# ilyakurdyukov/jpeg-quantsmooth

Hardware: AMD Instinct MI355X
Metric: 8x8 blocks/s at q=3 niter=3 (higher is better)
Workload: dtype f32

## Files before the change

### jpeg-quantsmooth_amd/csrc/qs_kernels.hip

```cpp
#include <hip/hip_runtime.h>
#include <stdint.h>
#include <stdlib.h>
#include "qs_device.h"
#include "qs_devfn.h"



__device__ __forceinline__ void wave_lds_sync() {
  __builtin_amdgcn_fence(__ATOMIC_RELEASE, "wavefront");
  __builtin_amdgcn_wave_barrier();
  __builtin_amdgcn_fence(__ATOMIC_ACQUIRE, "wavefront");
}

__device__ __forceinline__ uint32_t mulc(uint32_t a, int c) {
  return (uint32_t)__mul24((int)a, c);
}

__device__ __forceinline__ uint32_t lshl13_add(uint32_t x, uint32_t b) {
  uint32_t r;
  asm("v_lshl_add_u32 %0, %1, 13, %2" : "=v"(r) : "v"(x), "v"(b));
  return r;
}

__device__ __forceinline__ void idct8(uint32_t (&v)[8], uint32_t bias) {
  uint32_t z1, z2, z3, z4, z5, t0, t1, t2, t3, e0, e1, e2, e3;
  z2 = v[2]; z3 = v[6];
  z1 = mulc(z2 + z3, 4433);
  asm volatile("" : "+v"(z1));
  t2 = z1 - mulc(z3, 15137);
  t3 = z1 + mulc(z2, 6270);
  t0 = lshl13_add(v[0] + v[4], bias);
  t1 = lshl13_add(v[0] - v[4], bias);
  e0 = t0 + t3; e3 = t0 - t3; e1 = t1 + t2; e2 = t1 - t2;
  t0 = v[7]; t1 = v[5]; t2 = v[3]; t3 = v[1];
  z1 = t0 + t3; z2 = t1 + t2; z3 = t0 + t2; z4 = t1 + t3;
  z5 = mulc(z3 + z4, 9633);
  asm volatile("" : "+v"(z5));
  t0 = mulc(t0, 2446);  t1 = mulc(t1, 16819);
  t2 = mulc(t2, 25172); t3 = mulc(t3, 12299);
  z1 = mulc(z1, 7373);  z2 = mulc(z2, 20995);
  z3 = mulc(z3, 16069); z4 = mulc(z4, 3196);
  z3 = z5 - z3; z4 = z5 - z4;
  t0 += z3 - z1; t1 += z4 - z2; t2 += z3 - z2; t3 += z4 - z1;
  v[0] = e0 + t3; v[7] = e0 - t3;
  v[1] = e1 + t2; v[6] = e1 - t2;
  v[2] = e2 + t1; v[5] = e2 - t1;
  v[3] = e3 + t0; v[4] = e3 - t0;
}

__device__ __forceinline__ void idct_pass1(uint32_t (&ws)[64]) {
#pragma unroll
  for (int x = 0; x < 8; ++x) {
    uint32_t col[8];
#pragma unroll
    for (int j = 0; j < 8; ++j) col[j] = ws[j * 8 + x];
    idct8(col, 1024u);
#pragma unroll
    for (int j = 0; j < 8; ++j) ws[j * 8 + x] = (uint32_t)((int32_t)col[j] >> 11);
  }
}

__device__ __forceinline__ void idct_pass2_row(uint32_t (&row)[8], int (&out)[8]) {
  idct8(row, 257u << 17);
#pragma unroll
  for (int j = 0; j < 8; ++j) {
    int z = (int32_t)row[j];
    z = min(max(z, 0), (256 << 18) - 1);
    out[j] = z >> 18;
  }
}

#define QS_PIX_BITS 0x45000000u
__device__ __forceinline__ void idct_pass2_row_f(uint32_t (&row)[8], float (&out)[8]) {
  idct8(row, 257u << 17);
#pragma unroll
  for (int j = 0; j < 8; ++j) {
    int z = (int32_t)row[j];
    z = min(max(z, 0), (256 << 18) - 1);
    out[j] = __builtin_bit_cast(float, __builtin_amdgcn_alignbit(QS_PIX_BITS >> 14, (uint32_t)z, 18));
  }
}
__device__ __forceinline__ float pix_from_byte(uint32_t v, int n) {
  return __builtin_bit_cast(float, QS_PIX_BITS | ((v >> (8 * n)) & 0xffu));
}

__device__ __forceinline__ void
store_pixel_row(uint8_t* __restrict__ org, int pitch, int y, const int (&o)[8], int bx, int by, int wblk, int hblk,
                int rep_top, int rep_bot) {
  uint2 pk;
  pk.x = (uint32_t)o[0] | ((uint32_t)o[1] << 8) | ((uint32_t)o[2] << 16) | ((uint32_t)o[3] << 24);
  pk.y = (uint32_t)o[4] | ((uint32_t)o[5] << 8) | ((uint32_t)o[6] << 16) | ((uint32_t)o[7] << 24);
  uint8_t* rp = org + (size_t)y * pitch;
  *reinterpret_cast<uint2*>(rp) = pk;
  const bool top = (y == 0 && by == 0 && rep_top), bot = (y == 7 && by == hblk - 1 && rep_bot);
  if (bx == 0) {
    rp[-1] = (uint8_t)o[0];
    if (top) rp[-1 - pitch] = (uint8_t)o[0];
    if (bot) rp[-1 + pitch] = (uint8_t)o[0];
  }
  if (bx == wblk - 1) {
    rp[8] = (uint8_t)o[7];
    if (top) rp[8 - pitch] = (uint8_t)o[7];
    if (bot) rp[8 + pitch] = (uint8_t)o[7];
  }
  if (top) *reinterpret_cast<uint2*>(rp - pitch) = pk;
  if (bot) *reinterpret_cast<uint2*>(rp + pitch) = pk;
}

__device__ __forceinline__ void
idct_ws_to_plane(uint32_t (&ws)[64], uint8_t* __restrict__ plane, int wblk, int hblk, int pitch,
                 int rep_top, int rep_bot, int blk) {
  const int by = blk / wblk, bx = blk - by * wblk;
  idct_pass1(ws);
  uint8_t* org = plane + (size_t)(by * 8 + 1) * pitch + QS_APRON_X + bx * 8;
#pragma unroll
  for (int y = 0; y < 8; ++y) {
    uint32_t row[8]; int o[8];
#pragma unroll
    for (int j = 0; j < 8; ++j) row[j] = ws[y * 8 + j];
    idct_pass2_row(row, o);
    store_pixel_row(org, pitch, y, o, bx, by, wblk, hblk, rep_top, rep_bot);
  }
}

__device__ __forceinline__ void
idct_wave_to_plane(const QsConsts* __restrict__ cst, int16_t* __restrict__ coef,
                   uint8_t* __restrict__ plane, int wblk, int hblk, int pitch,
                   int first, int defer, int rep_top, int rep_bot, int* __restrict__ status, int base, uint32_t* lds) {
  const int lane = threadIdx.x & 63;
  const int nblk = wblk * hblk;
  const int nvec = min(64, nblk - base) * 8;
  uint4* gsrc = reinterpret_cast<uint4*>(coef) + (size_t)base * 8;
  uint4 v[8];
#pragma unroll
  for (int j = 0; j < 8; ++j) {
    const int idx = j * 64 + lane;
    v[j] = make_uint4(0, 0, 0, 0);
    if (idx < nvec) v[j] = gsrc[idx];
  }
  if (first) {
    int q[8], bad = 0;
    qs_load_qraw8(cst, lane & 7, q);
#pragma unroll
    for (int j = 0; j < 8; ++j) v[j] = qs_dequant8<true>(v[j], q, bad);
    if (!defer) {
#pragma unroll
      for (int j = 0; j < 8; ++j) {
        const int idx = j * 64 + lane;
        if (idx < nvec) gsrc[idx] = v[j];
      }
    }
    if (bad) atomicOr(status, 1);
  }
  {
    const int m0 = (lane & 7) * 4;
#pragma unroll
    for (int j = 0; j < 8; ++j) {
      uint32_t* dst = lds + m0 * QS_LDS_PITCH + (j * 8 + (lane >> 3));
      dst[0] = v[j].x; dst[QS_LDS_PITCH] = v[j].y; dst[2 * QS_LDS_PITCH] = v[j].z; dst[3 * QS_LDS_PITCH] = v[j].w;
    }
  }
  wave_lds_sync();
  const uint32_t* col = lds + lane;
  uint32_t ws[64];
#pragma unroll
  for (int r = 0; r < 32; ++r) {
    const uint32_t d = col[r * QS_LDS_PITCH];
    ws[r * 2] = (uint32_t)(int32_t)(int16_t)(d & 0xffff);
    ws[r * 2 + 1] = (uint32_t)((int32_t)d >> 16);
  }
  if (base + lane < nblk) idct_ws_to_plane(ws, plane, wblk, hblk, pitch, rep_top, rep_bot, base + lane);
}

__global__ void __launch_bounds__(256)
qs_idct_plane_kernel(const QsConsts* __restrict__ cst, int16_t* __restrict__ coef,
                     uint8_t* __restrict__ plane, int wblk, int hblk, int pitch,
                     int first, int rep_top, int rep_bot, int* __restrict__ status) {
  __shared__ uint32_t lds_all[4][32 * QS_LDS_PITCH];
  const int wave = threadIdx.x >> 6;
  const int base = __builtin_amdgcn_readfirstlane((int)(blockIdx.x * 256 + wave * 64));
  if (base >= wblk * hblk) return;
  idct_wave_to_plane(cst, coef, plane, wblk, hblk, pitch, first & 1, first & 2, rep_top, rep_bot, status, base, lds_all[wave]);
}

__global__ void __launch_bounds__(256)
qs_idct_set_kernel(const QsPlaneSet set, int first) {
  __shared__ uint32_t lds_all[4][32 * QS_LDS_PITCH];
  const int wave = threadIdx.x >> 6;
  const int w = __builtin_amdgcn_readfirstlane((int)(blockIdx.x * 4 + wave));
  if (w >= set.wave0[set.n]) return;
  const int i = qs_set_find(set, w);
  const QsPlaneRef& r = set.ref[i];
  const int base = (w - set.wave0[i]) * 64;
  if (base >= r.wblk * r.hblk) return;
  idct_wave_to_plane(r.cst, r.coef, r.plane, r.wblk, r.hblk, r.pitch, first, r.mode & QS_PLANE_QUANT,
                     r.mode & QS_PLANE_REP_TOP, r.mode & QS_PLANE_REP_BOT, r.status, base, lds_all[wave]);
}



typedef int16_t __attribute__((may_alias)) lds_i16;
__device__ __forceinline__ int lds_coef(const uint32_t* col, int i) {
  const lds_i16* p = reinterpret_cast<const lds_i16*>(col + (i >> 1) * QS_LDS_PITCH) + (i & 1);
  return *p;
}
__device__ __forceinline__ void lds_set_coef(uint32_t* col, int i, int v) {
  lds_i16* p = reinterpret_cast<lds_i16*>(col + (i >> 1) * QS_LDS_PITCH) + (i & 1);
  *p = (lds_i16)v;
}

static_assert(QS_LDS_PITCH * 4 == 260, "the literal offsets below assume a 260-byte row pitch");
#define QS_LDS16_GROUP(BASE, W, N0, O) \
  asm volatile("ds_read_i16 %0, %16 offset:" #O "\n\tds_read_i16 %1, %16 offset:" #O "+2\n\t" \
               "ds_read_i16 %2, %16 offset:" #O "+260\n\tds_read_i16 %3, %16 offset:" #O "+262\n\t" \
               "ds_read_i16 %4, %16 offset:" #O "+520\n\tds_read_i16 %5, %16 offset:" #O "+522\n\t" \
               "ds_read_i16 %6, %16 offset:" #O "+780\n\tds_read_i16 %7, %16 offset:" #O "+782\n\t" \
               "ds_read_i16 %8, %16 offset:" #O "+1040\n\tds_read_i16 %9, %16 offset:" #O "+1042\n\t" \
               "ds_read_i16 %10, %16 offset:" #O "+1300\n\tds_read_i16 %11, %16 offset:" #O "+1302\n\t" \
               "ds_read_i16 %12, %16 offset:" #O "+1560\n\tds_read_i16 %13, %16 offset:" #O "+1562\n\t" \
               "ds_read_i16 %14, %16 offset:" #O "+1820\n\tds_read_i16 %15, %16 offset:" #O "+1822\n\t" \
               "s_waitcnt lgkmcnt(0)" \
               : "=&v"(W[(N0) + 0]), "=&v"(W[(N0) + 1]), "=&v"(W[(N0) + 2]), "=&v"(W[(N0) + 3]), \
                 "=&v"(W[(N0) + 4]), "=&v"(W[(N0) + 5]), "=&v"(W[(N0) + 6]), "=&v"(W[(N0) + 7]), \
                 "=&v"(W[(N0) + 8]), "=&v"(W[(N0) + 9]), "=&v"(W[(N0) + 10]), "=&v"(W[(N0) + 11]), \
                 "=&v"(W[(N0) + 12]), "=&v"(W[(N0) + 13]), "=&v"(W[(N0) + 14]), "=&v"(W[(N0) + 15]) \
               : "v"(BASE) : "memory")
__device__ __forceinline__ void lds_read_block_i16(const uint32_t* col, uint32_t (&ws)[64]) {
  typedef const __attribute__((address_space(3))) uint32_t* lds_ptr;
  const uint32_t a0 = (uint32_t)(uintptr_t)(lds_ptr)col;
  const uint32_t a1 = a0 + 8 * 260, a2 = a0 + 16 * 260, a3 = a0 + 24 * 260;
  QS_LDS16_GROUP(a0, ws, 0, 0);
  QS_LDS16_GROUP(a1, ws, 16, 0);
  QS_LDS16_GROUP(a2, ws, 32, 0);
  QS_LDS16_GROUP(a3, ws, 48, 0);
}
__device__ __forceinline__ void lds_read_block_i16_1(const uint32_t* col, uint32_t (&ws)[64]) {
  typedef const __attribute__((address_space(3))) uint32_t* lds_ptr;
  const uint32_t a0 = (uint32_t)(uintptr_t)(lds_ptr)col;
  QS_LDS16_GROUP(a0, ws, 0, 0);
  QS_LDS16_GROUP(a0, ws, 16, 2080);
  QS_LDS16_GROUP(a0, ws, 32, 4160);
  QS_LDS16_GROUP(a0, ws, 48, 6240);
}

#define QS_PIX_SCALE 0.000244140625f
#define QS_TERM_D(D, W) { \
    float u_ = __builtin_amdgcn_fmed3f(Rs - __builtin_fabsf(D), 0.0f, 1.0f); \
    float t_ = u_ * u_; \
    float x_ = (D) * t_; \
    float y_ = (W) * t_; \
    num = num + x_ * y_; \
    den = den + y_ * y_; }
#define QS_TERM(A, B, W) { float d_ = (A) - (B); QS_TERM_D(d_, W) }

typedef float qs_w16 __attribute__((ext_vector_type(16)));
typedef int qs_i4 __attribute__((ext_vector_type(4)));
#define QS_SWAIT(BUF) asm volatile("s_waitcnt lgkmcnt(0)" : "+s"(BUF) : : "memory")

#define QS_WAVES_PER_WG 4
#define QS_SMOOTH_MIN_WAVES 3
#define QS_RESIDENT_WG (256 * QS_SMOOTH_MIN_WAVES * 4 / QS_WAVES_PER_WG)
#define QS_PRIO_SLOW 3
#define QS_PRIO_TERMS 0

#define QS_TERM_OPT(COND, A, B, W) { float d_, t_; \
        asm volatile( \
          "s_cmp_lg_u32 %[c], 0\n\t" \
          "s_cbranch_scc1 1f\n\t" \
          "v_sub_f32 %[d], %[a], %[b]\n\t" \
          "v_sub_f32 %[t], %[r], |%[d]| clamp\n\t" \
          "v_mul_f32 %[t], %[t], %[t]\n\t" \
          "v_mul_f32 %[d], %[d], %[t]\n\t" \
          "v_mul_f32 %[t], %[w], %[t]\n\t" \
          "v_mul_f32 %[d], %[d], %[t]\n\t" \
          "v_add_f32 %[n], %[n], %[d]\n\t" \
          "v_mul_f32 %[d], %[t], %[t]\n\t" \
          "v_add_f32 %[e], %[e], %[d]\n" \
          "1:" \
          : [n] "+v"(num), [e] "+v"(den), [d] "=&v"(d_), [t] "=&v"(t_) \
          : [a] "v"(A), [b] "v"(B), [w] "s"(W), [r] "s"(Rs), [c] "s"(COND) : "scc"); }
#define QS_TERM_ASM(A, B, W) { float d_, t_; \
        asm volatile( \
          "v_sub_f32 %[d], %[a], %[b]\n\t" \
          "v_sub_f32 %[t], %[r], |%[d]| clamp\n\t" \
          "v_mul_f32 %[t], %[t], %[t]\n\t" \
          "v_mul_f32 %[d], %[d], %[t]\n\t" \
          "v_mul_f32 %[t], %[w], %[t]\n\t" \
          "v_mul_f32 %[d], %[d], %[t]\n\t" \
          "v_add_f32 %[n], %[n], %[d]\n\t" \
          "v_mul_f32 %[d], %[t], %[t]\n\t" \
          "v_add_f32 %[e], %[e], %[d]" \
          : [n] "+v"(num), [e] "+v"(den), [d] "=&v"(d_), [t] "=&v"(t_) \
          : [a] "v"(A), [b] "v"(B), [w] "s"(W), [r] "s"(Rs)); }

#define QS_TERM_D_ASM(D, W) { float d_, t_; \
        asm volatile( \
          "v_sub_f32 %[t], %[r], |%[a]| clamp\n\t" \
          "v_mul_f32 %[t], %[t], %[t]\n\t" \
          "v_mul_f32 %[d], %[a], %[t]\n\t" \
          "v_mul_f32 %[t], %[w], %[t]\n\t" \
          "v_mul_f32 %[d], %[d], %[t]\n\t" \
          "v_add_f32 %[n], %[n], %[d]\n\t" \
          "v_mul_f32 %[d], %[t], %[t]\n\t" \
          "v_add_f32 %[e], %[e], %[d]" \
          : [n] "+v"(num), [e] "+v"(den), [d] "=&v"(d_), [t] "=&v"(t_) \
          : [a] "v"(D), [w] "s"(W), [r] "s"(Rs)); }
#ifndef QS_HOIST_DIAG
#define QS_HOIST_DIAG 32
#endif
#ifndef QS_Q1_SKIP
#define QS_Q1_SKIP 1
#endif
#ifndef QS_STASH
#define QS_STASH 1
#endif
#define QS_X_STASH 0
#define QS_X_EDGE 8
#define QS_X_REB 16
#define QS_X_DWORDS 20
static_assert(QS_WAVES_PER_WG * (32 * QS_LDS_PITCH + QS_X_DWORDS * 64) * 4 <= 160 * 1024 / 3, "LDS budget of three workgroups per CU");
typedef unsigned long long __attribute__((address_space(3))) qs_lds_u64;
__device__ __forceinline__ void qs_lds_add64(qs_lds_u64* p, long long v) {
  __hip_atomic_fetch_add(p, (unsigned long long)v, __ATOMIC_RELAXED, __HIP_MEMORY_SCOPE_WAVEFRONT);
}
__device__ __forceinline__ qs_lds_u64* qs_xreb(const uint32_t* col, const uint32_t* lds, int n) {
  typedef const __attribute__((address_space(3))) uint32_t* lds_ptr;
  uint32_t a = (uint32_t)(uintptr_t)(lds_ptr)col;
  asm volatile("" : "+v"(a));
  const uint32_t b = (uint32_t)(uintptr_t)(lds_ptr)lds;
  return (qs_lds_u64*)(a * 2u - b + (uint32_t)((32 * QS_LDS_PITCH + (QS_X_REB + 2 * n) * 64) * 4));
}

#define QS_SMOOTH_KERNEL_NAME qs_smooth_plane_kernel
#include "qs_smooth_kernel.inc"
#undef QS_SMOOTH_KERNEL_NAME
#define QS_SMOOTH_KERNEL_NAME qs_smooth_set_kernel
#define QS_SMOOTH_SET 1
#include "qs_smooth_kernel.inc"
#undef QS_SMOOTH_KERNEL_NAME
#undef QS_SMOOTH_SET

#define QS_DP_KERNEL_NAME qs_smooth_dp_kernel
#include "qs_smooth_dp_kernel.inc"
#undef QS_DP_KERNEL_NAME
#define QS_DP_KERNEL_NAME qs_smooth_dp_set_kernel
#define QS_DP_SET 1
#include "qs_smooth_dp_kernel.inc"
#undef QS_DP_KERNEL_NAME
#undef QS_DP_SET

__global__ void __launch_bounds__(256)
qs_clamp_kernel(int16_t* __restrict__ coef, size_t nvec) {
  size_t i = (size_t)blockIdx.x * 256 + threadIdx.x;
  const size_t stride = (size_t)gridDim.x * 256;
  uint4* p = reinterpret_cast<uint4*>(coef);
  for (; i < nvec; i += stride) {
    uint4 v = p[i];
    uint32_t d[4] = {v.x, v.y, v.z, v.w};
#pragma unroll
    for (int c = 0; c < 4; ++c) {
      int lo = (int16_t)(d[c] & 0xffff), hi = (int32_t)d[c] >> 16;
      lo = min(max(lo, -1023), 1023); hi = min(max(hi, -1023), 1023);
      d[c] = ((uint32_t)lo & 0xffffu) | ((uint32_t)hi << 16);
    }
    p[i] = make_uint4(d[0], d[1], d[2], d[3]);
  }
}

__global__ void __launch_bounds__(256)
qs_dequant_kernel(const QsConsts* __restrict__ cst, int16_t* __restrict__ coef, size_t nvec) {
  size_t i = (size_t)blockIdx.x * 256 + threadIdx.x;
  const size_t stride = (size_t)gridDim.x * 256;
  uint4* p = reinterpret_cast<uint4*>(coef);
  for (; i < nvec; i += stride) {
    uint4 v = p[i];
    uint32_t d[4] = {v.x, v.y, v.z, v.w};
    const int j = (int)(i & 7);
#pragma unroll
    for (int c = 0; c < 4; ++c) {
      int lo = (int16_t)(d[c] & 0xffff), hi = (int32_t)d[c] >> 16;
      lo *= cst->qraw[j * 8 + c * 2]; hi *= cst->qraw[j * 8 + c * 2 + 1];
      d[c] = ((uint32_t)lo & 0xffffu) | ((uint32_t)hi << 16);
    }
    p[i] = make_uint4(d[0], d[1], d[2], d[3]);
  }
}

#include "qs_launch.h"

void qs_launch_idct_plane(const QsConsts* cst, int16_t* coef, uint8_t* plane, int wblk, int hblk,
                          int first, int rep_top, int rep_bot, int* status, hipStream_t s) {
  const int nblk = wblk * hblk;
  const int f = first == 3 ? 3 : first ? 1 : 0;
  hipLaunchKernelGGL(qs_idct_plane_kernel, dim3((nblk + 255) / 256), dim3(256), 0, s,
                     cst, coef, plane, wblk, hblk, qs_plane_pitch(wblk), f, rep_top, rep_bot, status);
}

#define QS_DP_WAVES 4
static int qs_dp_waves(int groups) {
  static const int on = [] { const char* v = getenv("QS_HIP_DP"); return v ? atoi(v) : 1; }();
  static const int lim = [] { const char* v = getenv("QS_HIP_DP_GROUPS"); return v ? atoi(v) : 768; }();
  static const int lim2 = [] { const char* v = getenv("QS_HIP_DP_GROUPS2"); return v ? atoi(v) : 1536; }();
  if (!on) return 0;
  return groups <= lim ? QS_DP_WAVES : groups <= lim2 ? 2 : 0;
}

void qs_launch_smooth_plane(const QsConsts* cst, int16_t* coef, const uint8_t* plane, uint8_t* plane_next, int rep_top, int rep_bot,
                            int wblk, int hblk, int diag, int rebalance, int final_clamp, int blk_begin, int blk_end, hipStream_t s) {
  const int n = blk_end - blk_begin;
  if (n <= 0) return;
  const int pitch = qs_plane_pitch(wblk);
  const int rep = (rep_top ? QS_PLANE_REP_TOP : 0) | (rep_bot ? QS_PLANE_REP_BOT : 0);
  if (const int nw = qs_dp_waves((n + 63) / 64)) {
    const dim3 g((n + 63) / 64), b(64 * nw);
#define QS_GO_DP(D, W) hipLaunchKernelGGL((qs_smooth_dp_kernel<D, W>), g, b, 0, s, cst, coef, plane, plane_next, rep, wblk, hblk, pitch, rebalance, final_clamp, blk_begin, blk_end)
    if (nw == 2) { if (diag) QS_GO_DP(true, 2); else QS_GO_DP(false, 2); }
    else if (diag) QS_GO_DP(true, QS_DP_WAVES); else QS_GO_DP(false, QS_DP_WAVES);
#undef QS_GO_DP
    return;
  }
  const int per_wg = 64 * QS_WAVES_PER_WG;
  const dim3 grid((n + per_wg - 1) / per_wg), block(per_wg);
#define QS_GO(K) hipLaunchKernelGGL(K, grid, block, 0, s, cst, coef, plane, plane_next, rep, wblk, hblk, pitch, rebalance, final_clamp, blk_begin, blk_end)
  if (diag) QS_GO(qs_smooth_plane_kernel<true>); else QS_GO(qs_smooth_plane_kernel<false>);
#undef QS_GO
}

void qs_launch_idct_set(const QsPlaneSet& set, int first, hipStream_t s) {
  const int nw = set.wave0[set.n];
  if (nw <= 0) return;
  hipLaunchKernelGGL(qs_idct_set_kernel, dim3((nw + 3) / 4), dim3(256), 0, s, set, first);
}

void qs_launch_smooth_set(const QsPlaneSet& set, int diag, int final_clamp, hipStream_t s) {
  const int nw = set.wave0[set.n];
  if (nw <= 0) return;
  if (const int dw = qs_dp_waves(nw)) {
    const dim3 g(nw), b(64 * dw);
#define QS_GO_DP(D, W) hipLaunchKernelGGL((qs_smooth_dp_set_kernel<D, W>), g, b, 0, s, set, final_clamp)
    if (dw == 2) { if (diag) QS_GO_DP(true, 2); else QS_GO_DP(false, 2); }
    else if (diag) QS_GO_DP(true, QS_DP_WAVES); else QS_GO_DP(false, QS_DP_WAVES);
#undef QS_GO_DP
    return;
  }
  const dim3 grid((nw + QS_WAVES_PER_WG - 1) / QS_WAVES_PER_WG), block(64 * QS_WAVES_PER_WG);
  if (diag) hipLaunchKernelGGL(qs_smooth_set_kernel<true>, grid, block, 0, s, set, final_clamp);
  else      hipLaunchKernelGGL(qs_smooth_set_kernel<false>, grid, block, 0, s, set, final_clamp);
}

void qs_launch_clamp(int16_t* coef, size_t nblk, hipStream_t s) {
  const size_t nvec = nblk * 8;
  const int grid = (int)((nvec + 255) / 256 < 8192 ? (nvec + 255) / 256 : 8192);
  hipLaunchKernelGGL(qs_clamp_kernel, dim3(grid ? grid : 1), dim3(256), 0, s, coef, nvec);
}

void qs_launch_dequant(const QsConsts* cst, int16_t* coef, size_t nblk, hipStream_t s) {
  const size_t nvec = nblk * 8;
  const int grid = (int)((nvec + 255) / 256 < 8192 ? (nvec + 255) / 256 : 8192);
  hipLaunchKernelGGL(qs_dequant_kernel, dim3(grid ? grid : 1), dim3(256), 0, s, cst, coef, nvec);
}
```

### jpeg-quantsmooth_amd/csrc/qs_smooth_kernel.inc

```
template <bool DIAG>
__global__ void __launch_bounds__(64 * QS_WAVES_PER_WG, QS_SMOOTH_MIN_WAVES)
#ifdef QS_SMOOTH_SET
QS_SMOOTH_KERNEL_NAME(const QsPlaneSet set, int final_clamp) {
  __shared__ __attribute__((aligned(16))) uint32_t lds_all[QS_WAVES_PER_WG][32 * QS_LDS_PITCH + (DIAG ? 0 : QS_X_DWORDS * 64)];
#if QS_STASH
  __shared__ uint32_t stash_all[QS_WAVES_PER_WG][2 * 8 * 64];
#endif
  const int lane = threadIdx.x & 63, wave = DIAG ? (int)(threadIdx.x >> 6) : __builtin_amdgcn_readfirstlane((int)(threadIdx.x >> 6));
  uint32_t* lds = lds_all[wave];
  uint32_t* col = lds + lane;
  const int gw = __builtin_amdgcn_readfirstlane((int)(blockIdx.x * QS_WAVES_PER_WG + wave));
  if (gw >= set.wave0[set.n]) return;
  const int pi = qs_set_find(set, gw);
  const QsConsts* __restrict__ cst = set.ref[pi].cst;
  int16_t* __restrict__ coef = set.ref[pi].coef;
  const uint8_t* __restrict__ plane = set.ref[pi].plane;
  const int wblk = set.ref[pi].wblk, hblk = set.ref[pi].hblk, pitch = set.ref[pi].pitch;
  const int rebalance = set.ref[pi].mode & QS_PLANE_REBALANCE;
  const int nblk = wblk * hblk;
  const int base = (gw - set.wave0[pi]) * 64;
  (void)hblk;
#else
QS_SMOOTH_KERNEL_NAME(const QsConsts* __restrict__ cst, int16_t* __restrict__ coef,
                       const uint8_t* __restrict__ plane, uint8_t* __restrict__ plane_next, int rep,
                       int wblk, int hblk, int pitch,
                       int rebalance, int final_clamp, int blk_begin, int blk_end) {
  __shared__ __attribute__((aligned(16))) uint32_t lds_all[QS_WAVES_PER_WG][32 * QS_LDS_PITCH + (DIAG ? 0 : QS_X_DWORDS * 64)];
#if QS_STASH
  __shared__ uint32_t stash_all[QS_WAVES_PER_WG][2 * 8 * 64];
#endif
  const int lane = threadIdx.x & 63, wave = DIAG ? (int)(threadIdx.x >> 6) : __builtin_amdgcn_readfirstlane((int)(threadIdx.x >> 6));
  uint32_t* lds = lds_all[wave];
  uint32_t* col = lds + lane;
  const int nblk = blk_end;
  const int base = blk_begin + (blockIdx.x * QS_WAVES_PER_WG + wave) * 64;
#endif
  if (base >= nblk) return;
  const int tail_prio = __builtin_amdgcn_readfirstlane(
      (gridDim.x > QS_RESIDENT_WG && blockIdx.x >= (gridDim.x / QS_RESIDENT_WG) * QS_RESIDENT_WG) ? 1 : 0);
  const int nvec = min(64, nblk - base) * 8;
#ifdef QS_STAGGER
  { unsigned hwid; asm volatile("s_getreg_b32 %0, hwreg(HW_REG_HW_ID)" : "=s"(hwid)); if (hwid & 1u) __builtin_amdgcn_s_sleep(QS_STAGGER); }
#endif

  uint4* gsrc = reinterpret_cast<uint4*>(coef) + (size_t)base * 8;
  uint32_t bigacc = 0;
#define QS_BIG_ACC(V) if constexpr (!DIAG) bigacc |= ((V).x ^ ((V).x << 1)) | ((V).y ^ ((V).y << 1)) | ((V).z ^ ((V).z << 1)) | ((V).w ^ ((V).w << 1))
#ifdef QS_SMOOTH_SET
  if (set.ref[pi].mode & QS_PLANE_QUANT) {
    const int m0 = (lane & 7) * 4;
    int q[8], unused = 0;
    qs_load_qraw8(cst, lane & 7, q);
#pragma unroll
    for (int j = 0; j < 8; ++j) {
      const int idx = j * 64 + lane;
      uint4 v = make_uint4(0, 0, 0, 0);
      if (idx < nvec) v = gsrc[idx];
      v = qs_dequant8<false>(v, q, unused);
      QS_BIG_ACC(v);
      uint32_t* dst = lds + m0 * QS_LDS_PITCH + (j * 8 + (lane >> 3));
      dst[0] = v.x; dst[QS_LDS_PITCH] = v.y; dst[2 * QS_LDS_PITCH] = v.z; dst[3 * QS_LDS_PITCH] = v.w;
    }
  } else
#endif
  {
    const int m0 = (lane & 7) * 4;
#pragma unroll
    for (int j = 0; j < 8; ++j) {
      const int idx = j * 64 + lane;
      uint4 v = make_uint4(0, 0, 0, 0);
      if (idx < nvec) v = gsrc[idx];
      QS_BIG_ACC(v);
      uint32_t* dst = lds + m0 * QS_LDS_PITCH + (j * 8 + (lane >> 3));
      dst[0] = v.x; dst[QS_LDS_PITCH] = v.y; dst[2 * QS_LDS_PITCH] = v.z; dst[3 * QS_LDS_PITCH] = v.w;
    }
  }

  const int blk = min(base + lane, nblk - 1);
  const int by = blk / wblk, bx = blk - by * wblk;
  const uint8_t* org = plane + (size_t)(by * 8 + 1) * pitch + QS_APRON_X + bx * 8;
  uint32_t edge[8];
  {
    const uint2 t = *reinterpret_cast<const uint2*>(org - pitch);
    const uint2 b = *reinterpret_cast<const uint2*>(org + (size_t)8 * pitch);
    edge[0] = t.x; edge[1] = t.y; edge[2] = b.x; edge[3] = b.y;
    uint32_t l[8], r[8];
#pragma unroll
    for (int y = 0; y < 8; ++y) {
      l[y] = org[(ptrdiff_t)y * pitch - 1];
      r[y] = org[(ptrdiff_t)y * pitch + 8];
    }
    edge[4] = l[0] | (l[1] << 8) | (l[2] << 16) | (l[3] << 24);
    edge[5] = l[4] | (l[5] << 8) | (l[6] << 16) | (l[7] << 24);
    edge[6] = r[0] | (r[1] << 8) | (r[2] << 16) | (r[3] << 24);
    edge[7] = r[4] | (r[5] << 8) | (r[6] << 16) | (r[7] << 24);
  }
  uint32_t* const xcol = col + 32 * QS_LDS_PITCH;
  if constexpr (!DIAG) {
#pragma unroll
    for (int e = 0; e < 8; ++e) xcol[(QS_X_EDGE + e) * 64] = edge[e];
    *qs_xreb(col, lds, 0) = 0; *qs_xreb(col, lds, 1) = 0;
  }
  wave_lds_sync();

  constexpr int TS = DIAG ? 272 : 160;
  float px[DIAG ? 64 : 1];
  float bd[32];
  constexpr int NH = DIAG ? QS_HOIST_DIAG : 1;
  float hd[NH];
  float dh[DIAG ? 1 : 56], dv[DIAG ? 1 : 56];

  int kfirst = 63;
#if QS_STASH
  int stash_hi = 0;
#endif
  uint32_t chg = 0;
  uint64_t chg_any = 0;
#undef QS_BIG_ACC
  const bool big_wave = !DIAG && __builtin_amdgcn_ballot_w64((bigacc & 0xC000C000u) != 0) != 0;
  long long reb_m0 = 0, reb_m1 = 0;
  const float* tabp = cst->tab;
  const int32_t* recp = &cst->rec[0][0];
  qs_w16 WA, WB;
  qs_i4 REC;
  qs_i4 RECN;
  asm volatile("s_load_dwordx4 %0, %2, %3\n\ts_load_dwordx16 %1, %4, %5\n\ts_waitcnt lgkmcnt(0)"
               : "=&s"(REC), "=&s"(WA) : "s"(recp), "s"(63u * 16u), "s"(tabp), "s"((uint32_t)63 * (TS * 4)) : "memory");
  RECN = REC;

#pragma unroll 1
  for (int g = 0; g < 14; ++g) {
    __builtin_amdgcn_s_setprio(QS_PRIO_SLOW);
    if (g == 0 || (DIAG ? __builtin_amdgcn_ballot_w64(chg != 0) != 0 : chg_any != 0)) {
      chg = 0;
      chg_any = 0;
      uint32_t ws[64];
      if constexpr (DIAG) lds_read_block_i16(col, ws); else lds_read_block_i16_1(col, ws);
#if QS_STASH
      {
        uint32_t* stash = DIAG ? stash_all[wave] + lane : xcol + QS_X_STASH * 64;
#pragma unroll
        for (int x = 0; x < 8; ++x) {
          uint32_t c[8];
          const bool low = x <= (DIAG ? 1 : 0), high = x >= (DIAG ? 6 : 7);
          const int slot = (x == 0 || x == 7) ? 0 : 1;
          bool reuse = false, store = false;
          if (low) { reuse = g >= 1 && g <= 7 - x; store = g == 0; }
          if (high) {
            const int fin = 15 - x;
            const bool have = (stash_hi >> (x - 6)) & 1;
            reuse = g >= fin && have; store = g >= fin && !have;
          }
          if ((low || high) && reuse) {
#pragma unroll
            for (int j = 0; j < 8; ++j) c[j] = stash[(slot * 8 + j) * 64];
          } else {
#pragma unroll
            for (int j = 0; j < 8; ++j) c[j] = ws[j * 8 + x];
            idct8(c, 1024u);
#pragma unroll
            for (int j = 0; j < 8; ++j) c[j] = (uint32_t)((int32_t)c[j] >> 11);
            if ((low || high) && store) {
#pragma unroll
              for (int j = 0; j < 8; ++j) stash[(slot * 8 + j) * 64] = c[j];
              if (high) stash_hi |= 1 << (x - 6);
            }
          }
#pragma unroll
          for (int j = 0; j < 8; ++j) ws[j * 8 + x] = c[j];
        }
      }
#else
      idct_pass1(ws);
#endif
      if constexpr (!DIAG) {
        float prev[8];
#pragma unroll
        for (int y = 0; y < 8; ++y) {
          uint32_t row[8]; float o[8];
#pragma unroll
          for (int j = 0; j < 8; ++j) row[j] = ws[y * 8 + j];
          idct_pass2_row_f(row, o);
#pragma unroll
          for (int x = 0; x < 7; ++x) dh[y * 7 + x] = o[x] - o[x + 1];
          if (y > 0) {
#pragma unroll
            for (int x = 0; x < 8; ++x) dv[(y - 1) * 8 + x] = prev[x] - o[x];
          }
          if (y == 0 || y == 7) {
            const uint32_t e0 = xcol[(QS_X_EDGE + (y ? 2 : 0)) * 64], e1 = xcol[(QS_X_EDGE + (y ? 3 : 1)) * 64];
#pragma unroll
            for (int x = 0; x < 8; ++x) bd[(y ? 8 : 0) + x] = o[x] - pix_from_byte(x < 4 ? e0 : e1, x & 3);
          }
          {
            const uint32_t el = xcol[(QS_X_EDGE + 4 + (y >> 2)) * 64], er = xcol[(QS_X_EDGE + 6 + (y >> 2)) * 64];
            bd[16 + y] = o[0] - pix_from_byte(el, y & 3);
            bd[24 + y] = o[7] - pix_from_byte(er, y & 3);
          }
#pragma unroll
          for (int x = 0; x < 8; ++x) prev[x] = o[x];
          __builtin_amdgcn_sched_barrier(0);
        }
      } else {
#pragma unroll
      for (int y = 0; y < 8; ++y) {
        uint32_t row[8]; float o[8];
#pragma unroll
        for (int j = 0; j < 8; ++j) row[j] = ws[y * 8 + j];
        idct_pass2_row_f(row, o);
#pragma unroll
        for (int j = 0; j < 8; ++j) px[y * 8 + j] = o[j];
      }
#pragma unroll
      for (int e = 0; e < 8; ++e) asm volatile("" : "+v"(edge[e]));
#pragma unroll
      for (int x = 0; x < 8; ++x) {
        bd[x]      = px[x]         - pix_from_byte(edge[0 + (x >> 2)], x & 3);
        bd[8 + x]  = px[56 + x]    - pix_from_byte(edge[2 + (x >> 2)], x & 3);
        bd[16 + x] = px[x * 8]     - pix_from_byte(edge[4 + (x >> 2)], x & 3);
        bd[24 + x] = px[x * 8 + 7] - pix_from_byte(edge[6 + (x >> 2)], x & 3);
      }
#pragma unroll
      for (int t = 0; t < NH; ++t) hd[t] = px[(t / 7) * 8 + t % 7] - px[(t / 7) * 8 + t % 7 + 1];
      }
    }
    const int len = min(g + 1, 15 - g);
    const int klast = max(kfirst - len + 1, 1);
#pragma unroll 1
    for (int k = kfirst; k >= klast; --k) {
      if constexpr (DIAG) {
#pragma unroll
        for (int p = 0; p < 64; ++p) asm volatile("" : "+v"(px[p]));
      }
      const int md = REC[3];
      const int x2k = (REC[0] >> 16) & 31, qk = REC[1] & 0xffff, x1k = REC[1] >> 16;
      const uint32_t lds_off = ((uint32_t)md >> QS_REC_LDS_SHIFT) & 0x3fffu;
      int rs_bits = REC[2];
      asm volatile("" : "+s"(rs_bits));
      const float Rs = __builtin_bit_cast(float, rs_bits);
      const uint32_t kb = (uint32_t)k * (TS * 4);
      const uint32_t kb_nxt = kb - (uint32_t)(TS * 4);
      const uint32_t kb_s = (uint32_t)__builtin_amdgcn_readfirstlane((int)kb);
      const uint32_t kb_nxt_s = (uint32_t)__builtin_amdgcn_readfirstlane((int)kb_nxt);
      const uint32_t next_first = kb_nxt + (((uint32_t)md >> QS_REC_NXT_SHIFT) & 0x100u);
      const uint32_t after_V = DIAG ? kb + 640u : next_first;
      const uint32_t after_B = (md & QS_REC_V_ANY) ? kb + 384u : after_V;
#if QS_Q1_SKIP
      if (__builtin_expect(md & QS_REC_Q1, 0)) {
        {
          const int c0 = *reinterpret_cast<lds_i16*>(reinterpret_cast<char*>(col) + lds_off);
          if constexpr (DIAG) {
            reb_m0 += (long long)(c0 * c0);
            reb_m1 += (long long)(c0 * c0);
          } else {
            qs_lds_u64* const xreb = qs_xreb(col, lds, 0);
            qs_lds_add64(xreb, (long long)(c0 * c0));
            qs_lds_add64(xreb + 64, (long long)(c0 * c0));
          }
        }
        asm volatile("s_load_dwordx16 %0, %2, %3\n\ts_load_dwordx4 %1, %4, %5\n\ts_waitcnt lgkmcnt(0)"
                     : "=&s"(WA), "=&s"(RECN)
                     : "s"(tabp), "s"((uint32_t)__builtin_amdgcn_readfirstlane((int)next_first)), "s"(recp),
                       "s"((uint32_t)(k - 1) * 16u) : "memory");
        REC = RECN;
      } else
#endif
      {
      float num = 0.0f, den = 0.0f;
      asm volatile("s_setprio %c1\n\ts_cmp_eq_u32 %0, 0\n\ts_cbranch_scc1 1f\n\ts_setprio %c2\n1:"
                   : : "s"(tail_prio), "i"(QS_PRIO_TERMS), "i"(QS_PRIO_TERMS + 1) : "scc");

#define QS_ROW_D(W, Y) { \
        _Pragma("unroll") for (int x = 0; x < 7; ++x) { \
          QS_TERM(px[(Y) * 8 + x], px[(Y) * 8 + x + 9], W[x]) \
          QS_TERM(px[(Y) * 8 + x + 1], px[(Y) * 8 + x + 8], W[8 + x]) } }
#define QS_EDGE16(W, J0) { \
        _Pragma("unroll") for (int j = 0; j < 16; ++j) { \
          if constexpr (DIAG) QS_TERM_D(bd[(J0) + j], W[j]) \
          else QS_TERM_D_ASM(bd[(J0) + j], W[j]) } }
#define QS_HOISTED_TERM(T, WT) else if ((T) < NH) QS_TERM_D_ASM(hd[(T) % NH], WT)
#define QS_ROWS_H_M(W, Y0, MODE) { \
        _Pragma("unroll") for (int yy = 0; yy < 2; ++yy) \
        _Pragma("unroll") for (int x = 0; x < 7; ++x) { \
          if (((MODE) == 2 && (x & 1)) || ((MODE) == 1 && x == 3)) {} \
          else if constexpr (!DIAG) QS_TERM_D_ASM(dh[((Y0) + yy) * 7 + x], W[yy * 8 + x]) \
          QS_HOISTED_TERM(((Y0) + yy) * 7 + x, W[yy * 8 + x]) \
          else QS_TERM_ASM(px[((Y0) + yy) * 8 + x], px[((Y0) + yy) * 8 + x + 1], W[yy * 8 + x]) } }
#define QS_ROWS_V_M(W, Y0, NY, MODE) { \
        _Pragma("unroll") for (int yy = 0; yy < (NY); ++yy) \
        _Pragma("unroll") for (int x = 0; x < 8; ++x) { \
          if (((MODE) == 2 && (((Y0) + yy) & 1)) || ((MODE) == 1 && (Y0) + yy == 3)) {} \
          else if constexpr (!DIAG) QS_TERM_D_ASM(dv[((Y0) + yy) * 8 + x], W[yy * 8 + x]) \
          else QS_TERM_ASM(px[((Y0) + yy) * 8 + x], px[((Y0) + yy) * 8 + x + 8], W[yy * 8 + x]) } }

      const uint32_t rec_next = (uint32_t)(k - 1) * 16u;
#define QS_ISSUE(NXT, BYTEOFF) \
      asm volatile("s_load_dwordx16 %0, %3, %4" : "=&s"(NXT), "+v"(num), "+v"(den) \
                   : "s"(tabp), "s"((uint32_t)__builtin_amdgcn_readfirstlane((int)(BYTEOFF))) : "memory")
#define QS_ISSUE_K(NXT, IMM) \
      asm volatile("s_load_dwordx16 %0, %3, %4 offset:%c5" : "=&s"(NXT), "+v"(num), "+v"(den) \
                   : "s"(tabp), "s"(kb_s), "i"(IMM) : "memory")
#define QS_LAND(NXT) asm volatile("s_waitcnt lgkmcnt(0)" : "+s"(NXT), "+v"(num), "+v"(den) : : "memory")
#define QS_ISSUE_R(NXT, BYTEOFF) \
      asm volatile("s_load_dwordx16 %0, %4, %5\n\ts_load_dwordx4 %1, %6, %7" : "=&s"(NXT), "=&s"(RECN), "+v"(num), "+v"(den) \
                   : "s"(tabp), "s"((uint32_t)__builtin_amdgcn_readfirstlane((int)(BYTEOFF))), "s"(recp), "s"(rec_next) : "memory")
#define QS_LAND_R(NXT) asm volatile("s_waitcnt lgkmcnt(0)" : "+s"(NXT), "+s"(RECN), "+v"(num), "+v"(den) : : "memory")
#define QS_T4(O) "s_load_dword %1, %4, %5 offset:" #O "\n\ts_load_dword %1, %4, %5 offset:" #O "+0x40\n\ts_load_dword %1, %4, %5 offset:" #O "+0x80\n\ts_load_dword %1, %4, %5 offset:" #O "+0xc0\n\t"
#define QS_ISSUE_T(NXT, IMM) \
      uint32_t touch; \
      if (DIAG) asm volatile("s_load_dwordx16 %0, %4, %6 offset:%c7\n\t" QS_T4(0x0) QS_T4(0x100) QS_T4(0x200) QS_T4(0x300) "s_load_dword %1, %4, %5 offset:0x400" \
                   : "=&s"(NXT), "=&s"(touch), "+v"(num), "+v"(den) \
                   : "s"(tabp), "s"(kb_nxt_s), "s"(kb_s), "i"(IMM) : "memory"); \
      else      asm volatile("s_load_dwordx16 %0, %4, %6 offset:%c7\n\t" QS_T4(0x0) QS_T4(0x100) "s_load_dword %1, %4, %5 offset:0x200\n\ts_load_dword %1, %4, %5 offset:0x240" \
                   : "=&s"(NXT), "=&s"(touch), "+v"(num), "+v"(den) \
                   : "s"(tabp), "s"(kb_nxt_s), "s"(kb_s), "i"(IMM) : "memory")
#define QS_LAND_T(NXT) asm volatile("s_waitcnt lgkmcnt(0)" : "+s"(NXT), "+s"(touch), "+v"(num), "+v"(den) : : "memory")
#define QS_H_SECTION(MODE) { \
        QS_ISSUE_K(WB, 64);  QS_ROWS_H_M(WA, 0, MODE) QS_LAND(WB); \
        QS_ISSUE_K(WA, 128); QS_ROWS_H_M(WB, 2, MODE) QS_LAND(WA); \
        QS_ISSUE_K(WB, 192); QS_ROWS_H_M(WA, 4, MODE) QS_LAND(WB); \
        QS_ISSUE_K(WA, 256); QS_ROWS_H_M(WB, 6, MODE) QS_LAND(WA); }
      if (md & QS_REC_H_ANY) {
        if (md & QS_REC_H_SKIP4) QS_H_SECTION(2)
        else if (md & QS_REC_H_EVEN) QS_H_SECTION(1)
        else QS_H_SECTION(0)
      }
      QS_ISSUE_T(WB, 320); QS_EDGE16(WA, 0) QS_LAND_T(WB);
      if (!DIAG && !(md & QS_REC_V_ANY)) { QS_ISSUE_R(WA, after_B); QS_EDGE16(WB, 16) QS_LAND_R(WA); }
      else                   { QS_ISSUE(WA, after_B);   QS_EDGE16(WB, 16) QS_LAND(WA); }
#define QS_V_SECTION(MODE) { \
        QS_ISSUE_K(WB, 448); QS_ROWS_V_M(WA, 0, 2, MODE) QS_LAND(WB); \
        QS_ISSUE_K(WA, 512); QS_ROWS_V_M(WB, 2, 2, MODE) QS_LAND(WA); \
        QS_ISSUE_K(WB, 576); QS_ROWS_V_M(WA, 4, 2, MODE) QS_LAND(WB); \
        if (!DIAG) { QS_ISSUE_R(WA, after_V); QS_ROWS_V_M(WB, 6, 1, MODE) QS_LAND_R(WA); } \
        else       { QS_ISSUE(WA, after_V);   QS_ROWS_V_M(WB, 6, 1, MODE) QS_LAND(WA); } }
      if (md & QS_REC_V_ANY) {
        if (md & QS_REC_V_SKIP4) QS_V_SECTION(2)
        else if (md & QS_REC_V_EVEN) QS_V_SECTION(1)
        else QS_V_SECTION(0)
      }
      if (DIAG) {
        QS_ISSUE_K(WB, 704);  QS_ROW_D(WA, 0) QS_LAND(WB);
        QS_ISSUE_K(WA, 768);  QS_ROW_D(WB, 1) QS_LAND(WA);
        QS_ISSUE_K(WB, 832);  QS_ROW_D(WA, 2) QS_LAND(WB);
        QS_ISSUE_K(WA, 896);  QS_ROW_D(WB, 3) QS_LAND(WA);
        QS_ISSUE_K(WB, 960);  QS_ROW_D(WA, 4) QS_LAND(WB);
        QS_ISSUE_K(WA, 1024); QS_ROW_D(WB, 5) QS_LAND(WA);
        QS_ISSUE_R(WB, next_first); QS_ROW_D(WA, 6) QS_LAND_R(WB);
        WA = WB;
      }
#undef QS_ROWS_H_M
#undef QS_HOISTED_TERM
#undef QS_ROWS_V_M
#undef QS_H_SECTION
#undef QS_V_SECTION
#undef QS_ISSUE
#undef QS_ISSUE_K
#undef QS_LAND
#undef QS_ISSUE_R
#undef QS_LAND_R
#undef QS_ISSUE_T
#undef QS_LAND_T
#undef QS_T4

      __builtin_amdgcn_s_setprio(QS_PRIO_SLOW);
      lds_i16* const cptr = reinterpret_cast<lds_i16*>(reinterpret_cast<char*>(col) + lds_off);
      const int c0 = *cptr;
      const int r = f2i_x86(round_half_away((num / den) * 4096.0f));
      {
        int orig, lo, hi;
        interval(c0, qk, x1k, x2k, orig, lo, hi);
        int v = (int)((uint32_t)c0 - (uint32_t)r);
        v = min(max(v, lo), hi);
        if constexpr (DIAG) {
          *cptr = (lds_i16)v;
          chg |= (uint32_t)(v ^ c0);
          if (rebalance) {
            reb_m0 += (long long)(v * orig);
            reb_m1 += (long long)(orig * orig);
          }
        } else {
          if (__builtin_expect(big_wave, 0)) { asm volatile("" : "+v"(v)); v = r ? v : c0; }
          *cptr = (lds_i16)v;
          chg_any |= __builtin_amdgcn_ballot_w64(v != c0);
          if (rebalance) {
            qs_lds_u64* const xreb = qs_xreb(col, lds, 0);
            qs_lds_add64(xreb, (long long)(v * orig));
            qs_lds_add64(xreb + 64, (long long)(orig * orig));
          }
        }
      }
      REC = RECN;
      }
    }
    kfirst = klast - 1;
  }
  QS_SWAIT(WA);

  if (rebalance) {
    long long m0 = DIAG ? reb_m0 : (long long)*qs_xreb(col, lds, 0), m1 = DIAG ? reb_m1 : (long long)*qs_xreb(col, lds, 1);
    const bool big = big_wave;
    if (big) {
      m0 = 0; m1 = 0;
#pragma unroll 1
      for (int n = 1; n < 64; ++n) {
        const int c = lds_coef(col, n);
        int orig, lo, hi;
        interval(c, cst->qn[n], cst->x1n[n], cst->x2n[n], orig, lo, hi);
        m0 += (long long)(c * orig);
        m1 += (long long)(orig * orig);
      }
    }
    if (m1 > m0) {
      const int mul = (int)(((m1 << 13) + (m0 >> 1)) / m0);
#pragma unroll 9
      for (int n = 1; n < 64; ++n) {
        const int c = lds_coef(col, n);
        int orig, lo, hi;
        interval(c, cst->qn[n], cst->x1n[n], cst->x2n[n], orig, lo, hi);
        if (big) {
          const int div = cst->qn[n], a = (int16_t)orig;
          hi = a + (a < 0 ? div >> 1 : (div - 1) >> 1);
          lo = a - (a > 0 ? div >> 1 : (div - 1) >> 1);
        }
        int v = (c * mul + 0x1000) >> 13;
        v = min(max(v, lo), hi);
        lds_set_coef(col, n, v);
      }
    }
  }
  wave_lds_sync();

  {
    int lane2 = DIAG ? lane : (int)__builtin_amdgcn_mbcnt_hi(~0u, __builtin_amdgcn_mbcnt_lo(~0u, 0u));
    asm volatile("" : "+v"(lane2));
    const int lane = lane2;
    const int m0 = (lane & 7) * 4;
#pragma unroll
    for (int j = 0; j < 8; ++j) {
      const int idx = j * 64 + lane;
      const uint32_t* s = lds + m0 * QS_LDS_PITCH + (j * 8 + (lane >> 3));
      uint32_t d[4] = {s[0], s[QS_LDS_PITCH], s[2 * QS_LDS_PITCH], s[3 * QS_LDS_PITCH]};
      if (final_clamp) {
#pragma unroll
        for (int c = 0; c < 4; ++c) {
          int lo = (int16_t)(d[c] & 0xffff), hi = (int32_t)d[c] >> 16;
          lo = min(max(lo, -1023), 1023); hi = min(max(hi, -1023), 1023);
          d[c] = ((uint32_t)lo & 0xffffu) | ((uint32_t)hi << 16);
        }
      }
      if (idx < nvec) gsrc[idx] = make_uint4(d[0], d[1], d[2], d[3]);
    }
  }

#ifdef QS_SMOOTH_SET
  int pi2 = pi;
  asm volatile("" : "+s"(pi2));
  uint8_t* __restrict__ plane_next = set.ref[pi2].plane_next;
  const int rep = set.ref[pi2].mode, wblk2 = set.ref[pi2].wblk, hblk2 = set.ref[pi2].hblk, pitch2 = set.ref[pi2].pitch;
#else
  const int wblk2 = wblk, hblk2 = hblk, pitch2 = pitch;
#endif
  if (plane_next) {
    uint32_t ws[64];
    if constexpr (DIAG) lds_read_block_i16(col, ws); else lds_read_block_i16_1(col, ws);
    int lane3 = DIAG ? lane : (int)__builtin_amdgcn_mbcnt_hi(~0u, __builtin_amdgcn_mbcnt_lo(~0u, 0u));
    if constexpr (!DIAG) asm volatile("" : "+v"(lane3));
    if (base + lane3 < nblk)
      idct_ws_to_plane(ws, plane_next, wblk2, hblk2, pitch2, rep & QS_PLANE_REP_TOP, rep & QS_PLANE_REP_BOT, base + lane3);
  }
}

#undef QS_ROW_D
#undef QS_EDGE16
```

Baseline: 280.4 million.

## Keep rebalance sums in 32-bit registers and reload top/bottom edges per pass

In the non-diagonal kernel, the rebalance accumulators move from wavefront-scope 64-bit LDS atomics to 32-bit per-lane registers. The big-wave threshold is widened so that any lane that could overflow 32 bits falls back to the exact 64-bit recomputation. Top and bottom edge rows are no longer stashed in LDS; they are re-read from global memory at the start of each active pass from a stored offset, and the stash range widens to the diagonal pattern. The goal is to remove LDS atomics and edge traffic and free LDS dwords, at the cost of extra global loads per pass and reliance on the overflow guard.

```diff
diff --git a/jpeg-quantsmooth_amd/csrc/qs_kernels.hip b/jpeg-quantsmooth_amd/csrc/qs_kernels.hip
--- a/jpeg-quantsmooth_amd/csrc/qs_kernels.hip
+++ b/jpeg-quantsmooth_amd/csrc/qs_kernels.hip
@@ -315,21 +315,10 @@
 #define QS_STASH 1
 #endif
 #define QS_X_STASH 0
-#define QS_X_EDGE 8
-#define QS_X_REB 16
+#define QS_X_EDGE 16
 #define QS_X_DWORDS 20
+static_assert(QS_X_STASH + 16 <= QS_X_EDGE && QS_X_EDGE + 4 <= QS_X_DWORDS, "the lane's dwords behind the columns do not overlap");
 static_assert(QS_WAVES_PER_WG * (32 * QS_LDS_PITCH + QS_X_DWORDS * 64) * 4 <= 160 * 1024 / 3, "LDS budget of three workgroups per CU");
-typedef unsigned long long __attribute__((address_space(3))) qs_lds_u64;
-__device__ __forceinline__ void qs_lds_add64(qs_lds_u64* p, long long v) {
-  __hip_atomic_fetch_add(p, (unsigned long long)v, __ATOMIC_RELAXED, __HIP_MEMORY_SCOPE_WAVEFRONT);
-}
-__device__ __forceinline__ qs_lds_u64* qs_xreb(const uint32_t* col, const uint32_t* lds, int n) {
-  typedef const __attribute__((address_space(3))) uint32_t* lds_ptr;
-  uint32_t a = (uint32_t)(uintptr_t)(lds_ptr)col;
-  asm volatile("" : "+v"(a));
-  const uint32_t b = (uint32_t)(uintptr_t)(lds_ptr)lds;
-  return (qs_lds_u64*)(a * 2u - b + (uint32_t)((32 * QS_LDS_PITCH + (QS_X_REB + 2 * n) * 64) * 4));
-}
 
 #define QS_SMOOTH_KERNEL_NAME qs_smooth_plane_kernel
 #include "qs_smooth_kernel.inc"
diff --git a/jpeg-quantsmooth_amd/csrc/qs_smooth_kernel.inc b/jpeg-quantsmooth_amd/csrc/qs_smooth_kernel.inc
--- a/jpeg-quantsmooth_amd/csrc/qs_smooth_kernel.inc
+++ b/jpeg-quantsmooth_amd/csrc/qs_smooth_kernel.inc
@@ -80,10 +80,16 @@
   const int by = blk / wblk, bx = blk - by * wblk;
   const uint8_t* org = plane + (size_t)(by * 8 + 1) * pitch + QS_APRON_X + bx * 8;
   uint32_t edge[8];
+  uint32_t nrow8 = 0;
   {
-    const uint2 t = *reinterpret_cast<const uint2*>(org - pitch);
-    const uint2 b = *reinterpret_cast<const uint2*>(org + (size_t)8 * pitch);
-    edge[0] = t.x; edge[1] = t.y; edge[2] = b.x; edge[3] = b.y;
+    if constexpr (DIAG) {
+      const uint2 t = *reinterpret_cast<const uint2*>(org - pitch);
+      const uint2 b = *reinterpret_cast<const uint2*>(org + (size_t)8 * pitch);
+      edge[0] = t.x; edge[1] = t.y; edge[2] = b.x; edge[3] = b.y;
+    } else {
+      nrow8 = (uint32_t)(((size_t)(by * 8) * pitch + QS_APRON_X + bx * 8) >> 3);
+      edge[0] = edge[1] = edge[2] = edge[3] = 0;
+    }
     uint32_t l[8], r[8];
 #pragma unroll
     for (int y = 0; y < 8; ++y) {
@@ -98,8 +104,7 @@
   uint32_t* const xcol = col + 32 * QS_LDS_PITCH;
   if constexpr (!DIAG) {
 #pragma unroll
-    for (int e = 0; e < 8; ++e) xcol[(QS_X_EDGE + e) * 64] = edge[e];
-    *qs_xreb(col, lds, 0) = 0; *qs_xreb(col, lds, 1) = 0;
+    for (int e = 0; e < 4; ++e) xcol[(QS_X_EDGE + e) * 64] = edge[4 + e];
   }
   wave_lds_sync();
 
@@ -117,8 +122,9 @@
   uint32_t chg = 0;
   uint64_t chg_any = 0;
 #undef QS_BIG_ACC
-  const bool big_wave = !DIAG && __builtin_amdgcn_ballot_w64((bigacc & 0xC000C000u) != 0) != 0;
+  const bool big_wave = !DIAG && __builtin_amdgcn_ballot_w64((bigacc & 0xE000E000u) != 0) != 0;
   long long reb_m0 = 0, reb_m1 = 0;
+  uint32_t reb32_m0 = 0, reb32_m1 = 0;
   const float* tabp = cst->tab;
   const int32_t* recp = &cst->rec[0][0];
   qs_w16 WA, WB;
@@ -135,6 +141,23 @@
       chg = 0;
       chg_any = 0;
       uint32_t ws[64];
+      uint2 nbr_t = make_uint2(0, 0), nbr_b = make_uint2(0, 0);
+      if constexpr (!DIAG) {
+#ifdef QS_SMOOTH_SET
+        int pi3 = pi;
+        asm volatile("" : "+s"(pi3));
+        const uint8_t* const plane3 = set.ref[pi3].plane;
+        const int pitch3 = set.ref[pi3].pitch;
+#else
+        const uint8_t* const plane3 = plane;
+        const int pitch3 = pitch;
+#endif
+        uint32_t o8 = nrow8;
+        asm volatile("" : "+v"(o8));
+        const uint8_t* const above = plane3 + (size_t)o8 * 8;
+        nbr_t = *reinterpret_cast<const uint2*>(above);
+        nbr_b = *reinterpret_cast<const uint2*>(above + (size_t)9 * pitch3);
+      }
       if constexpr (DIAG) lds_read_block_i16(col, ws); else lds_read_block_i16_1(col, ws);
 #if QS_STASH
       {
@@ -142,7 +165,7 @@
 #pragma unroll
         for (int x = 0; x < 8; ++x) {
           uint32_t c[8];
-          const bool low = x <= (DIAG ? 1 : 0), high = x >= (DIAG ? 6 : 7);
+          const bool low = x <= 1, high = x >= 6;
           const int slot = (x == 0 || x == 7) ? 0 : 1;
           bool reuse = false, store = false;
           if (low) { reuse = g >= 1 && g <= 7 - x; store = g == 0; }
@@ -188,12 +211,12 @@
             for (int x = 0; x < 8; ++x) dv[(y - 1) * 8 + x] = prev[x] - o[x];
           }
           if (y == 0 || y == 7) {
-            const uint32_t e0 = xcol[(QS_X_EDGE + (y ? 2 : 0)) * 64], e1 = xcol[(QS_X_EDGE + (y ? 3 : 1)) * 64];
+            const uint32_t e0 = y ? nbr_b.x : nbr_t.x, e1 = y ? nbr_b.y : nbr_t.y;
 #pragma unroll
             for (int x = 0; x < 8; ++x) bd[(y ? 8 : 0) + x] = o[x] - pix_from_byte(x < 4 ? e0 : e1, x & 3);
           }
           {
-            const uint32_t el = xcol[(QS_X_EDGE + 4 + (y >> 2)) * 64], er = xcol[(QS_X_EDGE + 6 + (y >> 2)) * 64];
+            const uint32_t el = xcol[(QS_X_EDGE + (y >> 2)) * 64], er = xcol[(QS_X_EDGE + 2 + (y >> 2)) * 64];
             bd[16 + y] = o[0] - pix_from_byte(el, y & 3);
             bd[24 + y] = o[7] - pix_from_byte(er, y & 3);
           }
@@ -253,9 +276,8 @@
             reb_m0 += (long long)(c0 * c0);
             reb_m1 += (long long)(c0 * c0);
           } else {
-            qs_lds_u64* const xreb = qs_xreb(col, lds, 0);
-            qs_lds_add64(xreb, (long long)(c0 * c0));
-            qs_lds_add64(xreb + 64, (long long)(c0 * c0));
+            reb32_m0 += (uint32_t)(c0 * c0);
+            reb32_m1 += (uint32_t)(c0 * c0);
           }
         }
         asm volatile("s_load_dwordx16 %0, %2, %3\n\ts_load_dwordx4 %1, %4, %5\n\ts_waitcnt lgkmcnt(0)"
@@ -384,9 +406,8 @@
           *cptr = (lds_i16)v;
           chg_any |= __builtin_amdgcn_ballot_w64(v != c0);
           if (rebalance) {
-            qs_lds_u64* const xreb = qs_xreb(col, lds, 0);
-            qs_lds_add64(xreb, (long long)(v * orig));
-            qs_lds_add64(xreb + 64, (long long)(orig * orig));
+            reb32_m0 += (uint32_t)__mul24(v, orig);
+            reb32_m1 += (uint32_t)__mul24(orig, orig);
           }
         }
       }
@@ -398,7 +419,7 @@
   QS_SWAIT(WA);
 
   if (rebalance) {
-    long long m0 = DIAG ? reb_m0 : (long long)*qs_xreb(col, lds, 0), m1 = DIAG ? reb_m1 : (long long)*qs_xreb(col, lds, 1);
+    long long m0 = DIAG ? reb_m0 : (long long)(int32_t)reb32_m0, m1 = DIAG ? reb_m1 : (long long)(int32_t)reb32_m1;
     const bool big = big_wave;
     if (big) {
       m0 = 0; m1 = 0;
```

Result: no change. 281.8 million (median of 6 runs) (+0.5%).
